# nanoporetech/dorado

Measured on NVIDIA H100. Metric: basecalled samples/s, higher is better.
Workload: dtype f16 (fp32 accumulate; fp32 decode)

## Files before the change

### dorado_b200/csrc/decode.cu

```cuda
#include "decode.h"

#include "b200_crf_math.h"
#include "common.cuh"
#include "engine.h"
#include "nvtx.h"

#include <string>

namespace b200 {

namespace {

constexpr int kBeamW = 32;
constexpr uint32_t kCrcPoly = 0x82f63b78u;
constexpr uint32_t kCrcSeed = 0x12345678u;

template <int SL>
struct Dims {
    static constexpr int S = 1 << (2 * SL);
    static constexpr int C = 4 * S;
};

template <int SL>
struct ScanCfg {
// ... 28 lines not shown
    constexpr int RS = C / 4;
    float* out = bwd + (size_t)chunk_c * (T_pitch + 1) * S;
    const int q = v % P4, top = v / P4;
    const int st_row = 4 * (v & 3), st_col = v >> 2;

    uint2 pf[PF];
#pragma unroll
    for (int k = 0; k < PF; ++k) {
        const int tt = T - 1 - k;
        if (tt >= 0) pf[k] = __ldg(srow + (size_t)tt * RS);
    }
    auto stage = [&](int buf, const uint2& r) {
        const __half2 h0 = *reinterpret_cast<const __half2*>(&r.x), h1 = *reinterpret_cast<const __half2*>(&r.y);
        const float2 f0 = __half22float2(h0), f1 = __half22float2(h1);
        float* d = &st[g][buf][st_row * PITCH + st_col];
        d[0] = clampf(f0.x, clamp_val);
        d[PITCH] = clampf(f0.y, clamp_val);
        d[2 * PITCH] = clampf(f1.x, clamp_val);
        d[3 * PITCH] = clampf(f1.y, clamp_val);
    };
    float own = 0.0f;
    a[g][0][v] = 0.0f;
    if (active) out[(size_t)T * S + v] = 0.0f;
    stage(0, pf[0]);
    if (T - 1 - PF >= 0) pf[0] = __ldg(srow + (size_t)(T - 1 - PF) * RS);
    if constexpr (S <= 32) __syncwarp(); else named_bar_sync(1 + g, S);

    int cur = 0;
    for (int t = T - 1; t >= 0; t -= PF) {
#pragma unroll
        for (int k = 0; k < PF; ++k) {
            const int tt = t - k;
            if (tt >= 0) {
                if (tt - 1 >= 0) {
                    stage(cur ^ 1, pf[(k + 1) % PF]);
                    if (tt - 1 - PF >= 0) pf[(k + 1) % PF] = __ldg(srow + (size_t)(tt - 1 - PF) * RS);
                }
                const float4 nx = *reinterpret_cast<const float4*>(&a[g][cur][4 * q]);
                const float* sc = &st[g][cur][top * PITCH + q];
                own = b200_lse5(B200_ADD(own, blank), B200_ADD(nx.x, sc[0]), B200_ADD(nx.y, sc[4 * PITCH]),
                                B200_ADD(nx.z, sc[8 * PITCH]), B200_ADD(nx.w, sc[12 * PITCH]));
                a[g][cur ^ 1][v] = own;
                if (active) out[(size_t)tt * S + v] = own;
                if constexpr (S <= 32) __syncwarp(); else named_bar_sync(1 + g, S);
                cur ^= 1;
            }
        }
    }
}

__device__ __forceinline__ uint32_t crc_bits(uint32_t crc, uint32_t nb, int nbits) {
    for (int i = 0; i < nbits; ++i) {
        const uint32_t b = (nb ^ crc) & 1u;
        crc >>= 1;
        if (b) crc ^= kCrcPoly;
        nb >>= 1;
    }
    return crc;
}

__device__ __forceinline__ uint32_t crc2(uint32_t crc, uint32_t nb) {
    uint32_t b = (nb ^ crc) & 1u;
    crc = (crc >> 1) ^ (b ? kCrcPoly : 0u);
    b = ((nb >> 1) ^ crc) & 1u;
    crc = (crc >> 1) ^ (b ? kCrcPoly : 0u);
    return crc;
}

__device__ __forceinline__ uint32_t crc2_inv(uint32_t crc, uint32_t nb) {
    uint32_t b = crc >> 31;
    uint32_t t = crc ^ (b ? kCrcPoly : 0u);
    crc = (t << 1) | (b ^ ((nb >> 1) & 1u));
    b = crc >> 31;
    t = crc ^ (b ? kCrcPoly : 0u);
    crc = (t << 1) | (b ^ (nb & 1u));
    return crc;
}

constexpr int kHashSlots = 1024;

struct BeamSmem {
    __align__(16) float cand_score[5 * kBeamW];
    uint32_t cand_hash[5 * kBeamW];
    float new_score[kBeamW];
    uint32_t new_hash[kBeamW];
    uint32_t new_meta[kBeamW];
    __align__(16) uint32_t prev_hash[kBeamW];
    uint8_t slot_lane[kHashSlots];
};

struct BeamLane {
    uint32_t hash;
    uint32_t state;
    float score;
};

__device__ __forceinline__ uint32_t float_key(float f) {
    const uint32_t u = __float_as_uint(f);
    return (u & 0x80000000u) ? ~u : (u | 0x80000000u);
}

template <int SL>
__device__ int beam_init(const float* bw_row, BeamSmem& bs, BeamLane& me, int W, int lane) {
    constexpr int S = Dims<SL>::S;
    constexpr int VPL = S >= 32 ? S / 32 : 1;
    uint32_t keys[VPL];
#pragma unroll
    for (int j = 0; j < VPL; ++j) {
        const int s = lane * VPL + j;
        keys[j] = s < S ? float_key(bw_row[s]) : 0u;
    }
    uint32_t thr = 0u;
    if (W < S) {
        for (int bit = 31; bit >= 0; --bit) {
            const uint32_t cand = thr | (1u << bit);
            int c = 0;
#pragma unroll
            for (int j = 0; j < VPL; ++j) c += (lane * VPL + j < S) && (keys[j] >= cand);
            if (warp_sum_int(c) >= W) thr = cand;
        }
    }
    int c = 0;
#pragma unroll
    for (int j = 0; j < VPL; ++j) c += (lane * VPL + j < S) && (keys[j] >= thr);
    int incl = c;
#pragma unroll
    for (int o = 1; o < 32; o <<= 1) {
        const int v = __shfl_up_sync(0xffffffffu, incl, o);
        if (lane >= o) incl += v;
    }
    int pos = incl - c;
#pragma unroll
    for (int j = 0; j < VPL; ++j) {
        const int s = lane * VPL + j;
        if (s < S && keys[j] >= thr) {
            if (pos < W) bs.new_meta[pos] = (uint32_t)s;
            ++pos;
        }
    }
    __syncwarp();
    const int width = W < S ? W : S;
    if (lane < width) {
        me.state = bs.new_meta[lane] & 0xffffu;
        me.hash = crc_bits(kCrcSeed, me.state, 32);
        me.score = 0.0f;
    }
    __syncwarp();
    return width;
}

template <int SL>
__device__ __forceinline__ float kmer_block_prob(const float* post_row, int state) {
    constexpr int S = Dims<SL>::S;
    float prob = post_row[state];
    const int l = state >> 2;
    const int r = (state << 2) & (S - 1);
    constexpr int msb = S >> 2;
    const int d = l - r;
#pragma unroll
    for (int b = 0; b < 4; ++b) {
        const int L = l + msb * b, R = r + b;
        bool keepL = L != state;
#pragma unroll
        for (int bb = 0; bb < b; ++bb) keepL = keepL && (bb - msb * b != d);
        if (keepL) prob = B200_ADD(prob, post_row[L]);
        bool keepR = R != state;
#pragma unroll
        for (int bb = 0; bb <= b; ++bb) keepR = keepR && (b - msb * bb != d);
        if (keepR) prob = B200_ADD(prob, post_row[R]);
    }
    return prob < 0.0f ? 0.0f : (prob > 1.0f ? 1.0f : prob);
}

template <int SL>
__device__ int beam_step(const __half* sc_row,
                         const float* bw_row,
                         const float* post_row,
                         BeamSmem& bs,
                         BeamLane& me,
                         int width,
                         int W,
                         float log_beam_cut,
                         float blank,
                         bool last_block,
                         uint32_t* meta_row,
                         float* prob_row,
                         int lane,
                         long long* dbg) {
    constexpr int S = Dims<SL>::S;
    constexpr int SB = 2 * SL;
    if (dbg && lane == 0) dbg[0] = clock64();
    constexpr uint32_t mask = S - 1;
    const bool valid = lane < width;
    const uint32_t lt_mask = (1u << lane) - 1u;
    const uint32_t vmask = width >= 32 ? 0xffffffffu : ((1u << width) - 1u);

    uint32_t ns[4], hs[4];
    float s[5];
    float lmax = B200_FLT_LOWEST;
    const uint32_t latest = me.state & 3u;
    const uint32_t target = crc2_inv(me.hash, latest);
    const uint32_t own_slot = me.hash & (kHashSlots - 1);
    if (valid) {
        const uint32_t shifted = me.state << 2;
        const uint32_t dropped = shifted >> SB;
        const uint32_t nb = shifted & mask;
        const float4 bw4 = *reinterpret_cast<const float4*>(bw_row + nb);
        const float bws = bw_row[me.state];
        const float bwv[4] = {bw4.x, bw4.y, bw4.z, bw4.w};
        bs.slot_lane[own_slot] = (uint8_t)lane;
        bs.prev_hash[lane] = me.hash;
#pragma unroll
        for (uint32_t b = 0; b < 4; ++b) {
            ns[b] = nb | b;
            const uint32_t move_idx = ((ns[b] << 2) + dropped) & 0xffffu;
            s[b] = B200_ADD(B200_ADD(me.score, __half2float(sc_row[move_idx])), bwv[b]);
            hs[b] = crc2(me.hash, b);
            lmax = b200_fmaxf(lmax, s[b]);
        }
        s[4] = B200_ADD(B200_ADD(me.score, blank), bws);
        lmax = b200_fmaxf(lmax, s[4]);
        *reinterpret_cast<float4*>(&bs.cand_score[lane * 4]) = make_float4(s[0], s[1], s[2], s[3]);
    }
    float max_score = warp_max(lmax);
    __syncwarp();
    if (dbg && lane == 0) dbg[1] = clock64();

    int jm = -1;
    bool dup = false;
    {
        const uint32_t rb = valid ? bs.slot_lane[own_slot] : (uint32_t)lane;
        const uint32_t c = bs.slot_lane[target & (kHashSlots - 1)] & 31u;
        uint32_t ov = __ballot_sync(0xffffffffu, valid && rb != (uint32_t)lane);
        if (valid && ((vmask >> c) & 1u) && bs.prev_hash[c] == target) jm = (int)c;
        while (ov) {
            const int j = __ffs(ov) - 1;
            ov &= ov - 1;
            const uint32_t hj = __shfl_sync(0xffffffffu, me.hash, j);
            if (valid && lane != j && me.hash == hj) dup = true;
            if (valid && target == hj) jm = j;
        }
    }
    if (!__any_sync(0xffffffffu, dup)) {
        float folded = B200_FLT_LOWEST;
        if (jm >= 0) {
            const int pi = jm * 4 + (int)latest;
            const float st = s[4], sp = bs.cand_score[pi];
            folded = b200_log_sum_exp(st, sp);
            if (st > sp) {
                s[4] = folded;
                bs.cand_score[pi] = B200_FLT_LOWEST;
            } else {
                bs.cand_score[pi] = folded;
                s[4] = B200_FLT_LOWEST;
            }
        }
        max_score = b200_fmaxf(max_score, warp_max(folded));
        __syncwarp();
        if (valid) {
            const float4 r = *reinterpret_cast<const float4*>(&bs.cand_score[lane * 4]);
            s[0] = r.x; s[1] = r.y; s[2] = r.z; s[3] = r.w;
        }
    } else {
        if (valid) {
#pragma unroll
            for (int b = 0; b < 4; ++b) bs.cand_hash[lane * 4 + b] = hs[b];
            bs.cand_score[4 * width + lane] = s[4];
            bs.cand_hash[4 * width + lane] = me.hash;
        }
        bs.new_meta[lane] = valid ? latest : 0u;
        __syncwarp();
        float m2 = max_score;
        if (lane == 0) {
            for (int i = 0; i < width; ++i) {
                const int si = 4 * width + i;
                const int lt = (int)bs.new_meta[i];
                for (int j = 0; j < width; ++j) {
                    const int pi = j * 4 + lt;
                    if (bs.cand_hash[si] == bs.cand_hash[pi]) {
                        const float st = bs.cand_score[si], sp = bs.cand_score[pi];
                        const float folded = b200_log_sum_exp(st, sp);
                        if (st > sp) {
                            bs.cand_score[si] = folded;
                            bs.cand_score[pi] = B200_FLT_LOWEST;
                        } else {
                            bs.cand_score[pi] = folded;
                            bs.cand_score[si] = B200_FLT_LOWEST;
                        }
                        m2 = b200_fmaxf(m2, folded);
                    }
                }
            }
        }
        max_score = __shfl_sync(0xffffffffu, m2, 0);
        __syncwarp();
        if (valid) {
#pragma unroll
            for (int b = 0; b < 4; ++b) s[b] = bs.cand_score[lane * 4 + b];
            s[4] = bs.cand_score[4 * width + lane];
        }
        __syncwarp();
    }

    if (dbg && lane == 0) dbg[2] = clock64();
    auto count_part = [&](float c) {
        int n = 0;
        if (valid) {
#pragma unroll
            for (int k = 0; k < 5; ++k) n += (s[k] >= c);
        }
        return n;
    };
    float cutoff = B200_SUB(max_score, log_beam_cut);
    int cnt = warp_sum_int(count_part(cutoff));
    if (cnt > W) {
        const int min_w = (W * 8) / 10;
        float lo = cutoff, hi = max_score;
        int guesses = 1;
        while ((cnt > W || cnt < min_w) && guesses < 10) {
            if (cnt > W) {
                lo = cutoff;
                cutoff = B200_MUL(B200_ADD(cutoff, hi), 0.5f);
            } else {
                hi = cutoff;
                cutoff = B200_MUL(B200_ADD(cutoff, lo), 0.5f);
            }
            cnt = warp_sum_int(count_part(cutoff));
            ++guesses;
        }
        if (guesses == 10) {
            cutoff = hi;
            cnt = warp_sum_int(count_part(cutoff));
        }
        if (cnt > W) cnt = W;
    }

    if (dbg && lane == 0) dbg[3] = clock64();
    bool f[5];
#pragma unroll
    for (int k = 0; k < 5; ++k) f[k] = valid && (s[k] >= cutoff);
    const uint32_t b0 = __ballot_sync(0xffffffffu, f[0]), b1 = __ballot_sync(0xffffffffu, f[1]);
    const uint32_t b2 = __ballot_sync(0xffffffffu, f[2]), b3 = __ballot_sync(0xffffffffu, f[3]);
    const uint32_t b4 = __ballot_sync(0xffffffffu, f[4]);
    int pos = __popc(b0 & lt_mask) + __popc(b1 & lt_mask) + __popc(b2 & lt_mask) + __popc(b3 & lt_mask);
    const int steps_total = __popc(b0) + __popc(b1) + __popc(b2) + __popc(b3);
#pragma unroll
    for (int b = 0; b < 4; ++b) {
        if (f[b]) {
            if (pos < W) {
                bs.new_score[pos] = s[b];
                bs.new_hash[pos] = hs[b];
                bs.new_meta[pos] = ns[b] | ((uint32_t)lane << 16);
            }
            ++pos;
        }
    }
    if (f[4]) {
        const int sp = steps_total + __popc(b4 & lt_mask);
        if (sp < W) {
            bs.new_score[sp] = s[4];
            bs.new_hash[sp] = me.hash;
            bs.new_meta[sp] = me.state | ((uint32_t)lane << 16) | (1u << 24);
        }
    }
    __syncwarp();

    const bool nvalid = lane < cnt;
    uint32_t meta = 0;
    if (nvalid) {
        me.score = bs.new_score[lane];
        me.hash = bs.new_hash[lane];
        meta = bs.new_meta[lane];
        me.state = meta & 0xffffu;
    }

    if (dbg && lane == 0) dbg[4] = clock64();
    if (last_block) {
        const float best = warp_max(nvalid ? me.score : B200_FLT_LOWEST);
        const uint32_t eq = __ballot_sync(0xffffffffu, nvalid && me.score == best && best > B200_FLT_LOWEST);
        const int bi = eq ? (__ffs(eq) - 1) : 0;
        const int src = lane == 0 ? bi : (lane == bi ? 0 : lane);
        const float sc2 = __shfl_sync(0xffffffffu, me.score, src);
        const uint32_t h2 = __shfl_sync(0xffffffffu, me.hash, src);
        const uint32_t m2 = __shfl_sync(0xffffffffu, meta, src);
        me.score = sc2;
        me.hash = h2;
        meta = m2;
        me.state = meta & 0xffffu;
    }
    if (nvalid) {
        me.score = B200_SUB(me.score, bw_row[me.state]);
        meta_row[lane] = meta;
        prob_row[lane] = kmer_block_prob<SL>(post_row, (int)me.state);
    }
    __syncwarp();
    if (dbg && lane == 0) {
        dbg[5] = clock64();
        dbg[6] = cnt;
    }
    return cnt;
}

__device__ __forceinline__ void named_bar_arrive(int id, int nthreads) {
    asm volatile("bar.arrive %0, %1;" ::"r"(id), "r"(nthreads) : "memory");
}

template <int SL>
struct FwdCfg {
    using Scan = ScanCfg<SL>;
    static constexpr int GT = Scan::NT + 32;
    static constexpr int CH = GT <= 128 ? 2 : 1;
    static constexpr int THREADS = GT * CH;
};

template <int SL>
__global__ void __launch_bounds__(FwdCfg<SL>::THREADS) crf_fwd_beam_kernel(const __half* __restrict__ scores,
                                                                          const float* __restrict__ bwd,
                                                                          uint2* __restrict__ beam,
                                                                          int N,
                                                                          int T_pitch,
                                                                          float clamp_val,
                                                                          float blank,
                                                                          int W,
                                                                          float log_beam_cut,
                                                                          const int32_t* __restrict__ lens,
                                                                          int stride,
                                                                          long long* dbg) {
    using Cfg = ScanCfg<SL>;
    using F = FwdCfg<SL>;
    constexpr int S = Cfg::S, C = Cfg::C, P4 = Cfg::P4, SPT = Cfg::SPT, NT = Cfg::NT;
    constexpr int GT = F::GT, CH = F::CH;
    constexpr int NW = NT / 32;
    constexpr int PF = 4;

    const int g = threadIdx.x / GT;
    const int tid = threadIdx.x % GT;
    const int lane = threadIdx.x & 31;
    const int chunk = blockIdx.x * CH + g;
    const int BAR_SCAN = 1 + 5 * g, BAR_FULL = 2 + 5 * g, BAR_EMPTY = 4 + 5 * g;

    __shared__ __align__(16) float fa[CH][2][S];
    __shared__ __align__(16) __half sc_row[CH][2][C];
    __shared__ __align__(16) float bw_row[CH][2][S];
    __shared__ __align__(16) float post_row[CH][2][S];
    __shared__ float red[CH][2][NW];
    __shared__ BeamSmem bsm[CH];

    if (chunk >= N) return;
    const int T = lens ? min(T_pitch, __ldg(lens + chunk) / stride) : T_pitch;
    uint32_t* meta_out = reinterpret_cast<uint32_t*>(beam) + (size_t)chunk * T_pitch * kBeamW;
    float* prob_out = reinterpret_cast<float*>(beam) + ((size_t)N + chunk) * T_pitch * kBeamW;

    if (tid < NT) {
        const int v = tid;
        const int wv = v >> 5;
// ... 33 lines not shown
                    if (t >= 2) named_bar_sync(BAR_EMPTY + slot, GT);
                    if (d) d[9] = clock64();
                    float vsum[SPT];
                    float lmax = B200_FLT_LOWEST;
#pragma unroll
                    for (int e = 0; e < SPT; ++e) {
                        const uint2 r = pf[k][e];
                        const float bw = pb[k][e];
                        if (t + PF < T) {
                            pf[k][e] = __ldg(reinterpret_cast<const uint2*>(srow + (size_t)(t + PF) * C) + e);
                            pb[k][e] = __ldg(brow + (size_t)(t + PF + 1) * S + e);
                        }
                        const float2 f0 = __half22float2(*reinterpret_cast<const __half2*>(&r.x));
                        const float2 f1 = __half22float2(*reinterpret_cast<const __half2*>(&r.y));
                        const float s0 = clampf(f0.x, clamp_val), s1 = clampf(f0.y, clamp_val);
                        const float s2 = clampf(f1.x, clamp_val), s3 = clampf(f1.y, clamp_val);
                        const int st = SPT * v + e;
                        {
                            const __half2 c0 = __floats2half2_rn(s0, s1), c1 = __floats2half2_rn(s2, s3);
                            uint2 pk;
                            pk.x = *reinterpret_cast<const uint32_t*>(&c0);
                            pk.y = *reinterpret_cast<const uint32_t*>(&c1);
                            *reinterpret_cast<uint2*>(&sc_row[g][slot][4 * st]) = pk;
                        }
                        bw_row[g][slot][st] = bw;
                        const int p = st >> 2;
                        f[e] = b200_lse5(B200_ADD(f[e], blank), B200_ADD(fa[g][cur][p], s0), B200_ADD(fa[g][cur][p + P4], s1),
                                         B200_ADD(fa[g][cur][p + 2 * P4], s2), B200_ADD(fa[g][cur][p + 3 * P4], s3));
                        fa[g][cur ^ 1][st] = f[e];
                        vsum[e] = B200_ADD(f[e], bw);
                        lmax = b200_fmaxf(lmax, vsum[e]);
                    }
                    float mx = warp_max(lmax);
                    if constexpr (NW > 1) {
                        if (lane == 0) red[g][0][wv] = mx;
                        named_bar_sync(BAR_SCAN, NT);
                        mx = red[g][0][0];
#pragma unroll
                        for (int w = 1; w < NW; ++w) mx = b200_fmaxf(mx, red[g][0][w]);
                    }
                    float ex[SPT];
                    float part = 0.0f;
#pragma unroll
                    for (int e = 0; e < SPT; ++e) {
                        ex[e] = b200_expf_nonpos(B200_SUB(vsum[e], mx));
                        part = e == 0 ? ex[0] : B200_ADD(part, ex[e]);
                    }
#pragma unroll
                    for (int o = 16; o >= 1; o >>= 1) part = B200_ADD(part, __shfl_xor_sync(0xffffffffu, part, o));
                    float z = part;
                    if constexpr (NW > 1) {
                        if (lane == 0) red[g][1][wv] = part;
                        named_bar_sync(BAR_SCAN, NT);
                        z = red[g][1][0];
#pragma unroll
                        for (int w = 1; w < NW; ++w) z = B200_ADD(z, red[g][1][w]);
                    }
#pragma unroll
                    for (int e = 0; e < SPT; ++e) post_row[g][slot][SPT * v + e] = B200_DIV(ex[e], z);
                    named_bar_arrive(BAR_FULL + slot, GT);
                    if (d) d[10] = clock64();
                    cur ^= 1;
                }
            }
        }
    } else {
        named_bar_sync(BAR_SCAN, GT);
        BeamLane me{0u, 0u, 0.0f};
        int width = beam_init<SL>(bw_row[g][1], bsm[g], me, W, lane);
        named_bar_sync(BAR_SCAN, GT);
        for (int t = 0; t < T; ++t) {
            const int slot = t & 1;
            long long* d = (dbg && chunk == 0 && t >= 100 && t < 108) ? dbg + (t - 100) * 16 : nullptr;
            if (d && lane == 0) d[7] = clock64();
            named_bar_sync(BAR_FULL + slot, GT);
            width = beam_step<SL>(sc_row[g][slot], bw_row[g][slot], post_row[g][slot], bsm[g], me, width, W, log_beam_cut, blank,
                                  t == T - 1, meta_out + (size_t)t * kBeamW, prob_out + (size_t)t * kBeamW, lane, d);
            if (t + 2 < T) named_bar_arrive(BAR_EMPTY + slot, GT);
        }
    }
}

constexpr int kWarpDecodeMaxChunks = 16;
constexpr int kWarpStPitch = 16 + 2;

struct WarpDecodeSmem {
    __align__(16) float fa[2][64];
    float st[16 * kWarpStPitch];
    __align__(16) __half sc_row[256];
    __align__(16) float bw_row[64];
    __align__(16) float post_row[64];
    BeamSmem bs;
};

__device__ __forceinline__ float4 clamped_scores(const uint2& r, float clamp_val) {
    const float2 f0 = __half22float2(*reinterpret_cast<const __half2*>(&r.x));
    const float2 f1 = __half22float2(*reinterpret_cast<const __half2*>(&r.y));
    return make_float4(clampf(f0.x, clamp_val), clampf(f0.y, clamp_val), clampf(f1.x, clamp_val), clampf(f1.y, clamp_val));
}

__global__ void __launch_bounds__(kWarpDecodeMaxChunks * 32, 1) crf_decode_warp_kernel(const __half* __restrict__ scores,
                                                                                      float* __restrict__ bwd,
                                                                                      uint2* __restrict__ beam,
                                                                                      int N,
                                                                                      int T_pitch,
                                                                                      float clamp_val,
                                                                                      float blank,
                                                                                      int W,
                                                                                      float log_beam_cut,
                                                                                      const int32_t* __restrict__ lens,
                                                                                      int stride) {
    constexpr int S = Dims<3>::S, C = Dims<3>::C, P4 = S / 4, PITCH = kWarpStPitch;
    constexpr int RS = C / 4;
    constexpr int PF = 4;
    extern __shared__ __align__(16) unsigned char warp_decode_smem[];
    const int w = threadIdx.x >> 5, lane = threadIdx.x & 31;
    const int chunk = blockIdx.x * (blockDim.x >> 5) + w;
    if (chunk >= N) return;
    WarpDecodeSmem& sm = reinterpret_cast<WarpDecodeSmem*>(warp_decode_smem)[w];
    const int T = lens ? min(T_pitch, __ldg(lens + chunk) / stride) : T_pitch;
    const uint2* srow = reinterpret_cast<const uint2*>(scores + (size_t)chunk * T_pitch * C);
    float* brow = bwd + (size_t)chunk * (T_pitch + 1) * S;
    const int s0 = lane, s1 = lane + 32;

    {
        const int q = lane & 15, top = lane >> 4;
        auto stage = [&](const uint2& r, int v) {
            const float4 f = clamped_scores(r, clamp_val);
            float* d = &sm.st[4 * (v & 3) * PITCH + (v >> 2)];
            d[0] = f.x;
            d[PITCH] = f.y;
            d[2 * PITCH] = f.z;
            d[3 * PITCH] = f.w;
        };
        uint2 pf[PF][2];
#pragma unroll
        for (int k = 0; k < PF; ++k) {
            const int tt = T - 1 - k;
            if (tt >= 0) {
                pf[k][0] = __ldg(srow + (size_t)tt * RS + s0);
                pf[k][1] = __ldg(srow + (size_t)tt * RS + s1);
            }
        }
        float own0 = 0.0f, own1 = 0.0f;
        sm.fa[0][s0] = 0.0f;
        sm.fa[0][s1] = 0.0f;
        brow[(size_t)T * S + s0] = 0.0f;
        brow[(size_t)T * S + s1] = 0.0f;
        int cur = 0;
        for (int t = T - 1; t >= 0; t -= PF) {
#pragma unroll
            for (int k = 0; k < PF; ++k) {
                const int tt = t - k;
                if (tt >= 0) {
                    stage(pf[k][0], s0);
                    stage(pf[k][1], s1);
                    if (tt - PF >= 0) {
                        pf[k][0] = __ldg(srow + (size_t)(tt - PF) * RS + s0);
                        pf[k][1] = __ldg(srow + (size_t)(tt - PF) * RS + s1);
                    }
                    __syncwarp();
                    const float4 nx = *reinterpret_cast<const float4*>(&sm.fa[cur][4 * q]);
                    const float* sa = &sm.st[top * PITCH + q];
                    const float* sb = &sm.st[(top + 2) * PITCH + q];
                    own0 = b200_lse5(B200_ADD(own0, blank), B200_ADD(nx.x, sa[0]), B200_ADD(nx.y, sa[4 * PITCH]),
                                     B200_ADD(nx.z, sa[8 * PITCH]), B200_ADD(nx.w, sa[12 * PITCH]));
                    own1 = b200_lse5(B200_ADD(own1, blank), B200_ADD(nx.x, sb[0]), B200_ADD(nx.y, sb[4 * PITCH]),
                                     B200_ADD(nx.z, sb[8 * PITCH]), B200_ADD(nx.w, sb[12 * PITCH]));
                    sm.fa[cur ^ 1][s0] = own0;
                    sm.fa[cur ^ 1][s1] = own1;
                    brow[(size_t)tt * S + s0] = own0;
                    brow[(size_t)tt * S + s1] = own1;
                    __syncwarp();
                    cur ^= 1;
                }
            }
        }
    }
    __syncwarp();

    uint32_t* meta_out = reinterpret_cast<uint32_t*>(beam) + (size_t)chunk * T_pitch * kBeamW;
    float* prob_out = reinterpret_cast<float*>(beam) + ((size_t)N + chunk) * T_pitch * kBeamW;
    sm.fa[0][s0] = 0.0f;
    sm.fa[0][s1] = 0.0f;
    sm.bw_row[s0] = brow[s0];
    sm.bw_row[s1] = brow[s1];
    __syncwarp();
    BeamLane me{0u, 0u, 0.0f};
    int width = beam_init<3>(sm.bw_row, sm.bs, me, W, lane);
    uint2 r0n{}, r1n{};
    float b0n = 0.0f, b1n = 0.0f;
    if (T > 0) {
        r0n = __ldg(srow + s0);
        r1n = __ldg(srow + s1);
        b0n = brow[S + s0];
        b1n = brow[S + s1];
    }
    float f0 = 0.0f, f1 = 0.0f;
    int cur = 0;
    const int p0 = s0 >> 2, p1 = s1 >> 2;
    for (int t = 0; t < T; ++t) {
        const uint2 r0 = r0n, r1 = r1n;
        const float bw0 = b0n, bw1 = b1n;
        if (t + 1 < T) {
            r0n = __ldg(srow + (size_t)(t + 1) * RS + s0);
            r1n = __ldg(srow + (size_t)(t + 1) * RS + s1);
            b0n = brow[(size_t)(t + 2) * S + s0];
            b1n = brow[(size_t)(t + 2) * S + s1];
        }
        const float4 c0 = clamped_scores(r0, clamp_val), c1 = clamped_scores(r1, clamp_val);
        {
            const __half2 h00 = __floats2half2_rn(c0.x, c0.y), h01 = __floats2half2_rn(c0.z, c0.w);
            const __half2 h10 = __floats2half2_rn(c1.x, c1.y), h11 = __floats2half2_rn(c1.z, c1.w);
            *reinterpret_cast<uint2*>(&sm.sc_row[4 * s0]) =
                    make_uint2(*reinterpret_cast<const uint32_t*>(&h00), *reinterpret_cast<const uint32_t*>(&h01));
            *reinterpret_cast<uint2*>(&sm.sc_row[4 * s1]) =
                    make_uint2(*reinterpret_cast<const uint32_t*>(&h10), *reinterpret_cast<const uint32_t*>(&h11));
        }
        sm.bw_row[s0] = bw0;
        sm.bw_row[s1] = bw1;
        const float* fc = sm.fa[cur];
        f0 = b200_lse5(B200_ADD(f0, blank), B200_ADD(fc[p0], c0.x), B200_ADD(fc[p0 + P4], c0.y), B200_ADD(fc[p0 + 2 * P4], c0.z),
                       B200_ADD(fc[p0 + 3 * P4], c0.w));
        f1 = b200_lse5(B200_ADD(f1, blank), B200_ADD(fc[p1], c1.x), B200_ADD(fc[p1 + P4], c1.y), B200_ADD(fc[p1 + 2 * P4], c1.z),
                       B200_ADD(fc[p1 + 3 * P4], c1.w));
        sm.fa[cur ^ 1][s0] = f0;
        sm.fa[cur ^ 1][s1] = f1;
        const float v0 = B200_ADD(f0, bw0), v1 = B200_ADD(f1, bw1);
        const float mx = warp_max(b200_fmaxf(v0, v1));
        const float e0 = b200_expf_nonpos(B200_SUB(v0, mx)), e1 = b200_expf_nonpos(B200_SUB(v1, mx));
        float z0 = e0, z1 = e1;
#pragma unroll
        for (int o = 16; o >= 1; o >>= 1) {
            z0 = B200_ADD(z0, __shfl_xor_sync(0xffffffffu, z0, o));
            z1 = B200_ADD(z1, __shfl_xor_sync(0xffffffffu, z1, o));
        }
        const float z = B200_ADD(z0, z1);
        sm.post_row[s0] = B200_DIV(e0, z);
        sm.post_row[s1] = B200_DIV(e1, z);
        __syncwarp();
        width = beam_step<3>(sm.sc_row, sm.bw_row, sm.post_row, sm.bs, me, width, W, log_beam_cut, blank, t == T - 1,
                             meta_out + (size_t)t * kBeamW, prob_out + (size_t)t * kBeamW, lane, nullptr);
        cur ^= 1;
    }
}

int warp_decode_chunks_per_cta(int N, int runners) {
    const int R = runners > 1 ? runners : 1;
    const int per = (int)(((long long)N * R + kNumSMs - 1) / kNumSMs);
    return per < 1 ? 1 : (per > kWarpDecodeMaxChunks ? kWarpDecodeMaxChunks : per);
}

constexpr int kTbTile = 32;
constexpr int kTbWarps = 2;

__host__ __device__ constexpr size_t traceback_warp_bytes(int T) {
    return ((size_t)kTbTile * kBeamW * 4 + (size_t)((T + 3) & ~3) * (4 + 4 + 2) + 16 + 15) & ~(size_t)15;
}

__global__ void __launch_bounds__(kTbWarps * 32) crf_traceback_kernel(const uint32_t* __restrict__ beam_meta,
                                                                      const float* __restrict__ beam_prob,
                                                                      int N,
                                                                      int T_pitch,
                                                                      const int32_t* __restrict__ lens,
                                                                      int stride,
                                                                      const b200_qtable* __restrict__ qtable,
                                                                      uint8_t* __restrict__ moves_out,
                                                                      char* __restrict__ seq_out,
                                                                      char* __restrict__ qstr_out,
                                                                      int32_t* __restrict__ n_bases_out) {
    extern __shared__ __align__(16) unsigned char tb_smem[];
    __shared__ b200_qtable qt;
    for (int i = threadIdx.x; i < (int)(sizeof(b200_qtable) / 4); i += blockDim.x) {
        reinterpret_cast<uint32_t*>(&qt)[i] = reinterpret_cast<const uint32_t*>(qtable)[i];
    }
    __syncthreads();
    const int w = threadIdx.x >> 5, lane = threadIdx.x & 31;
    const int chunk = blockIdx.x * kTbWarps + w;
    if (chunk >= N) return;
    const int T = lens ? min(T_pitch, __ldg(lens + chunk) / stride) : T_pitch;
    const int Tp = (T_pitch + 3) & ~3;
    unsigned char* base = tb_smem + (size_t)w * traceback_warp_bytes(T_pitch);
    uint32_t* tile = reinterpret_cast<uint32_t*>(base);
    uint32_t* path = tile + kTbTile * kBeamW;
    float* pprob = reinterpret_cast<float*>(path + Tp);
    uint16_t* bstart = reinterpret_cast<uint16_t*>(pprob + Tp);

    const uint32_t* mrow = beam_meta + (size_t)chunk * T_pitch * kBeamW + lane;
    uint32_t nxt[kTbTile];
    auto load_tile = [&](int t_hi) {
        const int t_lo = t_hi - kTbTile;
#pragma unroll
        for (int r = 0; r < kTbTile; ++r) {
            const int t = t_lo + r;
            nxt[r] = t >= 0 ? __ldg(mrow + (size_t)t * kBeamW) : 0u;
        }
    };
    if (T > 0) load_tile(T);
    uint32_t ei = 0;
    for (int t_hi = T; t_hi > 0; t_hi -= kTbTile) {
#pragma unroll
        for (int r = 0; r < kTbTile; ++r) tile[r * kBeamW + lane] = nxt[r];
        __syncwarp();
        if (t_hi - kTbTile > 0) load_tile(t_hi - kTbTile);
        if (lane == 0) {
            const int t_lo = t_hi - kTbTile;
            const int r_lo = t_lo < 0 ? -t_lo : 0;
            for (int r = kTbTile - 1; r >= r_lo; --r) {
                const uint32_t e = tile[r * kBeamW + ei];
                path[t_lo + r] = (e & 0xffffu) | ((((e >> 24) & 1u) ^ 1u) << 16) | (ei << 24);
                ei = (e >> 16) & 0xffu;
            }
        }
        __syncwarp();
    }
    if (lane == 0 && T > 0) path[0] |= 1u << 16;
    __syncwarp();
    {
        const float* prow = beam_prob + (size_t)chunk * T_pitch * kBeamW;
        for (int t = lane; t < T; t += 32) {
            pprob[t] = b200_pow0p4f(__ldg(prow + (size_t)t * kBeamW + (path[t] >> 24)));
        }
    }
    __syncwarp();

    int nb = 0;
    for (int t0 = 0; t0 < T; t0 += 32) {
        const int t = t0 + lane;
        const bool m = t < T && ((path[t] >> 16) & 1u);
        const uint32_t bal = __ballot_sync(0xffffffffu, m);
        if (m) bstart[nb + __popc(bal & ((1u << lane) - 1u))] = (uint16_t)t;
        nb += __popc(bal);
    }
    if (lane == 0) bstart[nb] = (uint16_t)T;
    __syncwarp();

    uint8_t* mo = moves_out + (size_t)chunk * T_pitch;
    char* so = seq_out + (size_t)chunk * T_pitch;
    char* qo = qstr_out + (size_t)chunk * T_pitch;
    for (int t = lane; t < T_pitch; t += 32) mo[t] = t < T ? (uint8_t)((path[t] >> 16) & 1u) : 0;
    for (int p = lane; p < T_pitch; p += 32) {
        char sc = 0, qc = 0;
        if (p < nb) {
            const int b0 = bstart[p], b1 = bstart[p + 1];
            float bp = 0.0f, tp = 0.0f;
            int base = 0;
            for (int blk = b0; blk < b1; ++blk) {
                base = path[blk] & 3;
                const float prob = pprob[blk];
                const float wrong = B200_DIV(B200_SUB(1.0f, prob), 3.0f);
                bp = B200_ADD(bp, prob);
#pragma unroll
                for (int k = 0; k < 4; ++k) tp = B200_ADD(tp, k == base ? prob : wrong);
            }
            sc = "ACGT"[path[b0] & 3];
            qc = b200_qtable_lookup(&qt, bp, tp);
        }
        so[p] = sc;
        qo[p] = qc;
    }
    if (lane == 0) n_bases_out[chunk] = nb;
}

size_t traceback_smem_bytes(int T) { return kTbWarps * traceback_warp_bytes(T); }

void launch_traceback(const DecodeArgs& a, cudaStream_t stream, ProfileSink* prof) {
    const size_t smem = traceback_smem_bytes(a.T);
    if (smem > 48 * 1024) ensure_dynamic_smem(crf_traceback_kernel, 200 * 1024);
    const int grid = (a.N + kTbWarps - 1) / kTbWarps;
    NvtxRange r("decode");
    const uint32_t* meta = reinterpret_cast<const uint32_t*>(a.beam);
    const float* prob = reinterpret_cast<const float*>(a.beam) + (size_t)a.N * a.T * kBeamW;
    crf_traceback_kernel<<<grid, kTbWarps * 32, smem, stream>>>(meta, prob, a.N, a.T, a.lens, a.stride, a.qtable, a.moves,
                                                                a.sequence, a.qstring, a.n_bases);
    if (prof) prof->mark("crf_traceback", stream);
}

void launch_decode_warp(const DecodeArgs& a, cudaStream_t stream, ProfileSink* prof) {
    {
        const int cpc = warp_decode_chunks_per_cta(a.N, a.runners);
        const int grid = (a.N + cpc - 1) / cpc;
        const size_t smem = (size_t)cpc * sizeof(WarpDecodeSmem);
        ensure_dynamic_smem(crf_decode_warp_kernel, (int)(kWarpDecodeMaxChunks * sizeof(WarpDecodeSmem)));
        NvtxRange r("beam_search");
        crf_decode_warp_kernel<<<grid, cpc * 32, smem, stream>>>(a.scores, a.bwd, a.beam, a.N, a.T, a.clamp_val, a.blank,
                                                                 a.beam_width, a.log_beam_cut, a.lens, a.stride);
        if (prof) prof->mark("crf_fwd_beam", stream);
    }
    launch_traceback(a, stream, prof);
    B200_CUDA(cudaGetLastError());
}

template <int SL>
void launch_decode(const DecodeArgs& a, cudaStream_t stream, ProfileSink* prof) {
    {
        constexpr int S = Dims<SL>::S;
        constexpr int CH = S >= 256 ? 1 : 256 / S;
        const int grid = (a.N + CH - 1) / CH;
        NvtxRange r("back_guides");
        crf_bwd_scan_kernel<SL><<<grid, S * CH, 0, stream>>>(a.scores, a.bwd, a.N, a.T, a.clamp_val, a.blank, a.lens, a.stride);
        if (prof) prof->mark("crf_bwd_scan", stream);
    }
    {
        using F = FwdCfg<SL>;
        const int grid = (a.N + F::CH - 1) / F::CH;
        NvtxRange r("beam_search");
        crf_fwd_beam_kernel<SL><<<grid, F::THREADS, 0, stream>>>(a.scores, a.bwd, a.beam, a.N, a.T, a.clamp_val, a.blank,
                                                                   a.beam_width, a.log_beam_cut, a.lens, a.stride, a.dbg);
        if (prof) prof->mark("crf_fwd_beam", stream);
    }
    launch_traceback(a, stream, prof);
    B200_CUDA(cudaGetLastError());
}

}

size_t decode_max_blocks() {
    int T = 65535;
    while (traceback_smem_bytes(T) > 200 * 1024) T -= 64;
    return (size_t)T;
}

void carve_decode_scratch(Bump& b, int N, int T, int state_len, float** bwd, uint2** beam) {
    const size_t S = (size_t)1 << (2 * state_len);
    *bwd = b.take<float>((size_t)N * (T + 1) * S * sizeof(float));
    *beam = b.take<uint2>((size_t)N * T * kBeamW * sizeof(uint2));
}

int decode_launches(int state_len) { return state_len == 3 ? 2 : 3; }

void decode_scores(const DecodeArgs& a, cudaStream_t stream, ProfileSink* prof) {
    if (a.beam_width < 1 || a.beam_width > kBeamW) {
        throw std::invalid_argument("b200 decode: beam_width must be in [1, 32]");
    }
    if (a.T < 1 || a.T > 65535 || a.N < 1) {
        throw std::invalid_argument("b200 decode: need 1 <= T <= 65535 and N >= 1");
    }
    if (!a.qtable) throw std::invalid_argument("b200 decode: quality table missing");
    if (a.lens && a.stride < 1) throw std::invalid_argument("b200 decode: chunk lengths need the model stride");
    if (traceback_smem_bytes(a.T) > 200 * 1024) {
        throw std::invalid_argument("b200 decode: " + std::to_string(a.T) + " blocks per chunk exceed what the traceback kernel "
                                    "holds in shared memory (about 10 700); use a smaller chunk size");
    }
    switch (a.state_len) {
        case 3: launch_decode_warp(a, stream, prof); break;
        case 4: launch_decode<4>(a, stream, prof); break;
        case 5: launch_decode<5>(a, stream, prof); break;
        default: throw std::invalid_argument("b200 decode: state_len must be 3, 4 or 5");
    }
}

}
```

### include/b200_crf_math.h

```cpp
#ifndef B200_CRF_MATH_H
#define B200_CRF_MATH_H

#include <stdint.h>

#if defined(__CUDA_ARCH__)
#define B200_MATH_FN static __device__ __forceinline__
#define B200_FMA(a, b, c) __fmaf_rn((a), (b), (c))
#define B200_MUL(a, b) __fmul_rn((a), (b))
#define B200_ADD(a, b) __fadd_rn((a), (b))
#define B200_SUB(a, b) __fsub_rn((a), (b))
#define B200_DIV(a, b) __fdiv_rn((a), (b))
#define B200_F2U(x) __float_as_uint(x)
#define B200_U2F(x) __uint_as_float(x)
#else
#include <math.h>
#include <string.h>
#define B200_MATH_FN static inline
#define B200_FMA(a, b, c) fmaf((a), (b), (c))
#define B200_MUL(a, b) ((a) * (b))
#define B200_ADD(a, b) ((a) + (b))
#define B200_SUB(a, b) ((a) - (b))
#define B200_DIV(a, b) ((a) / (b))
static inline uint32_t b200_f2u_(float x) {
    uint32_t u;
    memcpy(&u, &x, 4);
    return u;
}
static inline float b200_u2f_(uint32_t u) {
    float x;
    memcpy(&x, &u, 4);
    return x;
}
#define B200_F2U(x) b200_f2u_(x)
#define B200_U2F(x) b200_u2f_(x)
#endif

#define B200_FLT_LOWEST (-3.402823466e+38f)

B200_MATH_FN float b200_fmaxf(float a, float b) { return a > b ? a : b; }

B200_MATH_FN float b200_expf(float x) {
    const float xc = x < -86.0f ? -86.0f : (x > 88.0f ? 88.0f : x);
    const float t = B200_MUL(xc, 1.44269504088896341f);
    const float big = 12582912.0f;
    const float tb = B200_ADD(t, big);
    const float n = B200_SUB(tb, big);
    float r = B200_FMA(n, -0.693359375f, xc);
    r = B200_FMA(n, 2.12194440e-4f, r);
    float p = 1.9875691500e-4f;
    p = B200_FMA(p, r, 1.3981999507e-3f);
    p = B200_FMA(p, r, 8.3334519073e-3f);
    p = B200_FMA(p, r, 4.1665795894e-2f);
    p = B200_FMA(p, r, 1.6666665459e-1f);
    p = B200_FMA(p, r, 5.0000001201e-1f);
    const float r2 = B200_MUL(r, r);
    p = B200_FMA(p, r2, r);
    p = B200_ADD(p, 1.0f);
    const float scale = B200_U2F((B200_F2U(tb) << 23) + 0x3f800000u);
    const float y = B200_MUL(p, scale);
    return x < -86.0f ? 0.0f : y;
}

B200_MATH_FN float b200_expf_nonpos(float x) {
    const float xc = x < -86.0f ? -86.0f : x;
    const float t = B200_MUL(xc, 1.44269504088896341f);
    const float big = 12582912.0f;
    const float tb = B200_ADD(t, big);
    const float n = B200_SUB(tb, big);
    float r = B200_FMA(n, -0.693359375f, xc);
    r = B200_FMA(n, 2.12194440e-4f, r);
    float p = 1.9875691500e-4f;
    p = B200_FMA(p, r, 1.3981999507e-3f);
    p = B200_FMA(p, r, 8.3334519073e-3f);
    p = B200_FMA(p, r, 4.1665795894e-2f);
    p = B200_FMA(p, r, 1.6666665459e-1f);
    p = B200_FMA(p, r, 5.0000001201e-1f);
    const float r2 = B200_MUL(r, r);
    p = B200_FMA(p, r2, r);
    p = B200_ADD(p, 1.0f);
    const float scale = B200_U2F((B200_F2U(tb) << 23) + 0x3f800000u);
    const float y = B200_MUL(p, scale);
    return x < -86.0f ? 0.0f : y;
}

B200_MATH_FN float b200_logf(float x) {
    const uint32_t ix = B200_F2U(x);
    int32_t e = (int32_t)((ix >> 23) & 0xffu) - 126;
    float m = B200_U2F((ix & 0x007fffffu) | 0x3f000000u);
    if (m < 0.707106781186547524f) {
        e -= 1;
        m = B200_SUB(B200_ADD(m, m), 1.0f);
    } else {
        m = B200_SUB(m, 1.0f);
    }
    const float z = B200_MUL(m, m);
    float y = 7.0376836292e-2f;
    y = B200_FMA(y, m, -1.1514610310e-1f);
    y = B200_FMA(y, m, 1.1676998740e-1f);
    y = B200_FMA(y, m, -1.2420140846e-1f);
    y = B200_FMA(y, m, 1.4249322787e-1f);
    y = B200_FMA(y, m, -1.6668057665e-1f);
    y = B200_FMA(y, m, 2.0000714765e-1f);
    y = B200_FMA(y, m, -2.4999993993e-1f);
    y = B200_FMA(y, m, 3.3333331174e-1f);
    y = B200_MUL(B200_MUL(y, m), z);
    const float fe = (float)e;
    y = B200_FMA(fe, -2.12194440e-4f, y);
    y = B200_FMA(z, -0.5f, y);
    float r = B200_ADD(m, y);
    r = B200_FMA(fe, 0.693359375f, r);
    return r;
}

B200_MATH_FN float b200_log1pf(float x) {
    const float u = B200_ADD(1.0f, x);
    const float c = B200_SUB(x, B200_SUB(u, 1.0f));
    return B200_ADD(b200_logf(u), B200_DIV(c, u));
}

B200_MATH_FN float b200_log_sum_exp(float x, float y) {
    const float d = B200_SUB(x, y);
    const float ad = d < 0.0f ? -d : d;
    const float mx = b200_fmaxf(x, y);
    if (ad < 17.0f) {
        return B200_ADD(mx, b200_log1pf(b200_expf(-ad)));
    }
    return mx;
}

B200_MATH_FN float b200_lse5(float v_stay, float v0, float v1, float v2, float v3) {
    float m = b200_fmaxf(v_stay, v0);
    m = b200_fmaxf(m, v1);
    m = b200_fmaxf(m, v2);
    m = b200_fmaxf(m, v3);
    float s = b200_expf_nonpos(B200_SUB(v_stay, m));
    s = B200_ADD(s, b200_expf_nonpos(B200_SUB(v0, m)));
    s = B200_ADD(s, b200_expf_nonpos(B200_SUB(v1, m)));
    s = B200_ADD(s, b200_expf_nonpos(B200_SUB(v2, m)));
    s = B200_ADD(s, b200_expf_nonpos(B200_SUB(v3, m)));
    return B200_ADD(m, b200_logf(s));
}

#if defined(__CUDA_ARCH__)
#define B200_DFMA(a, b, c) __fma_rn((a), (b), (c))
#define B200_DMUL(a, b) __dmul_rn((a), (b))
#define B200_DADD(a, b) __dadd_rn((a), (b))
#define B200_DSUB(a, b) __dsub_rn((a), (b))
#define B200_DDIV(a, b) __ddiv_rn((a), (b))
#define B200_D2U(x) ((uint64_t)__double_as_longlong(x))
#define B200_U2D(x) __longlong_as_double((long long)(x))
#define B200_D2F(x) __double2float_rn(x)
#else
#define B200_DFMA(a, b, c) fma((a), (b), (c))
#define B200_DMUL(a, b) ((a) * (b))
#define B200_DADD(a, b) ((a) + (b))
#define B200_DSUB(a, b) ((a) - (b))
#define B200_DDIV(a, b) ((a) / (b))
static inline uint64_t b200_d2u_(double x) {
    uint64_t u;
    memcpy(&u, &x, 8);
    return u;
}
static inline double b200_u2d_(uint64_t u) {
    double x;
    memcpy(&x, &u, 8);
    return x;
}
#define B200_D2U(x) b200_d2u_(x)
#define B200_U2D(x) b200_u2d_(x)
#define B200_D2F(x) ((float)(x))
#endif

B200_MATH_FN float b200_pow0p4f(float p) {
    if (p <= 0.0f) {
        return 0.0f;
    }
    if (p >= 1.0f) {
        return 1.0f;
    }
    const double x = (double)p;
    const uint64_t ix = B200_D2U(x);
    int64_t e = (int64_t)((ix >> 52) & 0x7ffu) - 1023;
    double m = B200_U2D((ix & 0x000fffffffffffffull) | 0x3ff0000000000000ull);
    if (m > 1.4142135623730951) {
        m = B200_DMUL(m, 0.5);
        e += 1;
    }
    const double s = B200_DDIV(B200_DSUB(m, 1.0), B200_DADD(m, 1.0));
    const double s2 = B200_DMUL(s, s);
    double q = 1.0 / 23.0;
    q = B200_DFMA(q, s2, 1.0 / 21.0);
    q = B200_DFMA(q, s2, 1.0 / 19.0);
    q = B200_DFMA(q, s2, 1.0 / 17.0);
    q = B200_DFMA(q, s2, 1.0 / 15.0);
    q = B200_DFMA(q, s2, 1.0 / 13.0);
    q = B200_DFMA(q, s2, 1.0 / 11.0);
    q = B200_DFMA(q, s2, 1.0 / 9.0);
    q = B200_DFMA(q, s2, 1.0 / 7.0);
    q = B200_DFMA(q, s2, 1.0 / 5.0);
    q = B200_DFMA(q, s2, 1.0 / 3.0);
    double lm = B200_DFMA(B200_DMUL(s, s2), q, s);
    lm = B200_DADD(lm, lm);
    const double fe = (double)e;
    double lx = B200_DFMA(fe, 1.90821492927058770002e-10, lm);
    lx = B200_DFMA(fe, 6.93147180369123816490e-01, lx);
    const double y = B200_DMUL(lx, 0.4000000059604644775390625);
    const double t = B200_DMUL(y, 1.44269504088896338700e+00);
    const double big = 6755399441055744.0;
    const double n = B200_DSUB(B200_DADD(t, big), big);
    double r = B200_DFMA(n, -6.93147180369123816490e-01, y);
    r = B200_DFMA(n, -1.90821492927058770002e-10, r);
    double ex = 1.0 / 6227020800.0;
    ex = B200_DFMA(ex, r, 1.0 / 479001600.0);
    ex = B200_DFMA(ex, r, 1.0 / 39916800.0);
    ex = B200_DFMA(ex, r, 1.0 / 3628800.0);
    ex = B200_DFMA(ex, r, 1.0 / 362880.0);
    ex = B200_DFMA(ex, r, 1.0 / 40320.0);
// ... 90 lines not shown
```

Before: 1.099 billion.

## Streamline CRF warp decode: register-resident backward scores, packed beam smem, half clamp

The backward pass now loads scores with 128-bit loads and uses byte_perm to pick each lane's pairs in registers. This drops the shared-memory transpose staging buffer and a per-step syncwarp. Beam candidates are packed into one uint4 array so each lane does a single vector store and load. The kernel is templated to clamp in half precision when the clamp value is exactly representable in fp16. Several micro-optimisations are bundled in: CRC hashes via linearity (crc2(h,0) xor crc2(0,b)), branch-free expf underflow via a -88 clamp, and hardware fmaxf in lse5. These risk small numerical differences, for example NaN handling in fmaxf and the tiny underflow values of expf.

Result: faster. 1.126 billion (median of 6 runs) (+2.5%).

```diff
diff --git a/dorado_b200/csrc/decode.cu b/dorado_b200/csrc/decode.cu
--- a/dorado_b200/csrc/decode.cu
+++ b/dorado_b200/csrc/decode.cu
@@ -134,9 +134,7 @@
 struct BeamSmem {
     __align__(16) float cand_score[5 * kBeamW];
     uint32_t cand_hash[5 * kBeamW];
-    float new_score[kBeamW];
-    uint32_t new_hash[kBeamW];
-    uint32_t new_meta[kBeamW];
+    uint4 kept[kBeamW];
     __align__(16) uint32_t prev_hash[kBeamW];
     uint8_t slot_lane[kHashSlots];
 };
@@ -186,14 +184,14 @@
     for (int j = 0; j < VPL; ++j) {
         const int s = lane * VPL + j;
         if (s < S && keys[j] >= thr) {
-            if (pos < W) bs.new_meta[pos] = (uint32_t)s;
+            if (pos < W) bs.kept[pos].z = (uint32_t)s;
             ++pos;
         }
     }
     __syncwarp();
     const int width = W < S ? W : S;
     if (lane < width) {
-        me.state = bs.new_meta[lane] & 0xffffu;
+        me.state = bs.kept[lane].z & 0xffffu;
         me.hash = crc_bits(kCrcSeed, me.state, 32);
         me.score = 0.0f;
     }
@@ -251,7 +249,8 @@
     float s[5];
     float lmax = B200_FLT_LOWEST;
     const uint32_t latest = me.state & 3u;
-    const uint32_t target = crc2_inv(me.hash, latest);
+    const uint32_t target = crc2_inv(me.hash, 0u) ^ latest;
+    const uint32_t hash0 = crc2(me.hash, 0u);
     const uint32_t own_slot = me.hash & (kHashSlots - 1);
     if (valid) {
         const uint32_t shifted = me.state << 2;
@@ -267,7 +266,7 @@
             ns[b] = nb | b;
             const uint32_t move_idx = ((ns[b] << 2) + dropped) & 0xffffu;
             s[b] = B200_ADD(B200_ADD(me.score, __half2float(sc_row[move_idx])), bwv[b]);
-            hs[b] = crc2(me.hash, b);
+            hs[b] = hash0 ^ crc2(0u, b);
             lmax = b200_fmaxf(lmax, s[b]);
         }
         s[4] = B200_ADD(B200_ADD(me.score, blank), bws);
@@ -320,13 +319,13 @@
             bs.cand_score[4 * width + lane] = s[4];
             bs.cand_hash[4 * width + lane] = me.hash;
         }
-        bs.new_meta[lane] = valid ? latest : 0u;
+        bs.kept[lane].z = valid ? latest : 0u;
         __syncwarp();
         float m2 = max_score;
         if (lane == 0) {
             for (int i = 0; i < width; ++i) {
                 const int si = 4 * width + i;
-                const int lt = (int)bs.new_meta[i];
+                const int lt = (int)bs.kept[i].z;
                 for (int j = 0; j < width; ++j) {
                     const int pi = j * 4 + lt;
                     if (bs.cand_hash[si] == bs.cand_hash[pi]) {
@@ -399,30 +398,23 @@
 #pragma unroll
     for (int b = 0; b < 4; ++b) {
         if (f[b]) {
-            if (pos < W) {
-                bs.new_score[pos] = s[b];
-                bs.new_hash[pos] = hs[b];
-                bs.new_meta[pos] = ns[b] | ((uint32_t)lane << 16);
-            }
+            if (pos < W) bs.kept[pos] = make_uint4(__float_as_uint(s[b]), hs[b], ns[b] | ((uint32_t)lane << 16), 0u);
             ++pos;
         }
     }
     if (f[4]) {
         const int sp = steps_total + __popc(b4 & lt_mask);
-        if (sp < W) {
-            bs.new_score[sp] = s[4];
-            bs.new_hash[sp] = me.hash;
-            bs.new_meta[sp] = me.state | ((uint32_t)lane << 16) | (1u << 24);
-        }
+        if (sp < W) bs.kept[sp] = make_uint4(__float_as_uint(s[4]), me.hash, me.state | ((uint32_t)lane << 16) | (1u << 24), 0u);
     }
     __syncwarp();
 
     const bool nvalid = lane < cnt;
     uint32_t meta = 0;
     if (nvalid) {
-        me.score = bs.new_score[lane];
-        me.hash = bs.new_hash[lane];
-        meta = bs.new_meta[lane];
+        const uint4 k = bs.kept[lane];
+        me.score = __uint_as_float(k.x);
+        me.hash = k.y;
+        meta = k.z;
         me.state = meta & 0xffffu;
     }
 
@@ -622,23 +614,50 @@
 }
 
 constexpr int kWarpDecodeMaxChunks = 16;
-constexpr int kWarpStPitch = 16 + 2;
 
 struct WarpDecodeSmem {
     __align__(16) float fa[2][64];
-    float st[16 * kWarpStPitch];
     __align__(16) __half sc_row[256];
     __align__(16) float bw_row[64];
     __align__(16) float post_row[64];
     BeamSmem bs;
 };
 
-__device__ __forceinline__ float4 clamped_scores(const uint2& r, float clamp_val) {
-    const float2 f0 = __half22float2(*reinterpret_cast<const __half2*>(&r.x));
-    const float2 f1 = __half22float2(*reinterpret_cast<const __half2*>(&r.y));
-    return make_float4(clampf(f0.x, clamp_val), clampf(f0.y, clamp_val), clampf(f1.x, clamp_val), clampf(f1.y, clamp_val));
-}
-
+__device__ __forceinline__ __half2 half_clamp_bound(float clamp_val) {
+    return __float2half2_rn(clamp_val > 0.0f ? clamp_val : __int_as_float(0x7f800000));
+}
+
+template <bool kHalfClamp>
+__device__ __forceinline__ float2 clamp_pair(uint32_t w, float clamp_val, __half2 bound) {
+    __half2 h = *reinterpret_cast<const __half2*>(&w);
+    if constexpr (kHalfClamp) {
+        return __half22float2(__hmin2(__hmax2(h, __hneg2(bound)), bound));
+    } else {
+        const float2 f = __half22float2(h);
+        return make_float2(clampf(f.x, clamp_val), clampf(f.y, clamp_val));
+    }
+}
+
+template <bool kHalfClamp>
+__device__ __forceinline__ float4 clamp_scores(uint2& r, float clamp_val, __half2 bound) {
+    __half2 h0 = *reinterpret_cast<const __half2*>(&r.x), h1 = *reinterpret_cast<const __half2*>(&r.y);
+    if constexpr (kHalfClamp) {
+        h0 = __hmin2(__hmax2(h0, __hneg2(bound)), bound);
+        h1 = __hmin2(__hmax2(h1, __hneg2(bound)), bound);
+        r = make_uint2(*reinterpret_cast<const uint32_t*>(&h0), *reinterpret_cast<const uint32_t*>(&h1));
+        const float2 f0 = __half22float2(h0), f1 = __half22float2(h1);
+        return make_float4(f0.x, f0.y, f1.x, f1.y);
+    } else {
+        const float2 f0 = __half22float2(h0), f1 = __half22float2(h1);
+        const float4 c = make_float4(clampf(f0.x, clamp_val), clampf(f0.y, clamp_val), clampf(f1.x, clamp_val),
+                                     clampf(f1.y, clamp_val));
+        const __half2 c0 = __floats2half2_rn(c.x, c.y), c1 = __floats2half2_rn(c.z, c.w);
+        r = make_uint2(*reinterpret_cast<const uint32_t*>(&c0), *reinterpret_cast<const uint32_t*>(&c1));
+        return c;
+    }
+}
+
+template <bool kHalfClamp>
 __global__ void __launch_bounds__(kWarpDecodeMaxChunks * 32, 1) crf_decode_warp_kernel(const __half* __restrict__ scores,
                                                                                       float* __restrict__ bwd,
                                                                                       uint2* __restrict__ beam,
@@ -650,7 +669,7 @@
                                                                                       float log_beam_cut,
                                                                                       const int32_t* __restrict__ lens,
                                                                                       int stride) {
-    constexpr int S = Dims<3>::S, C = Dims<3>::C, P4 = S / 4, PITCH = kWarpStPitch;
+    constexpr int S = Dims<3>::S, C = Dims<3>::C, P4 = S / 4;
     constexpr int RS = C / 4;
     constexpr int PF = 4;
     extern __shared__ __align__(16) unsigned char warp_decode_smem[];
@@ -662,24 +681,21 @@
     const uint2* srow = reinterpret_cast<const uint2*>(scores + (size_t)chunk * T_pitch * C);
     float* brow = bwd + (size_t)chunk * (T_pitch + 1) * S;
     const int s0 = lane, s1 = lane + 32;
+    const __half2 bound = half_clamp_bound(clamp_val);
 
     {
         const int q = lane & 15, top = lane >> 4;
-        auto stage = [&](const uint2& r, int v) {
-            const float4 f = clamped_scores(r, clamp_val);
-            float* d = &sm.st[4 * (v & 3) * PITCH + (v >> 2)];
-            d[0] = f.x;
-            d[PITCH] = f.y;
-            d[2 * PITCH] = f.z;
-            d[3 * PITCH] = f.w;
-        };
-        uint2 pf[PF][2];
+        const uint4* qrow = reinterpret_cast<const uint4*>(srow) + 2 * q;
+        constexpr int RQ = C / 8;
+        const uint32_t sel = top ? 0x7632u : 0x5410u;
+        auto pair = [&](uint32_t lo, uint32_t hi) { return clamp_pair<kHalfClamp>(__byte_perm(lo, hi, sel), clamp_val, bound); };
+        uint4 pf[PF][2];
 #pragma unroll
         for (int k = 0; k < PF; ++k) {
             const int tt = T - 1 - k;
             if (tt >= 0) {
-                pf[k][0] = __ldg(srow + (size_t)tt * RS + s0);
-                pf[k][1] = __ldg(srow + (size_t)tt * RS + s1);
+                pf[k][0] = __ldg(qrow + (size_t)tt * RQ);
+                pf[k][1] = __ldg(qrow + (size_t)tt * RQ + 1);
             }
         }
         float own0 = 0.0f, own1 = 0.0f;
@@ -687,26 +703,24 @@
         sm.fa[0][s1] = 0.0f;
         brow[(size_t)T * S + s0] = 0.0f;
         brow[(size_t)T * S + s1] = 0.0f;
+        __syncwarp();
         int cur = 0;
         for (int t = T - 1; t >= 0; t -= PF) {
 #pragma unroll
             for (int k = 0; k < PF; ++k) {
                 const int tt = t - k;
                 if (tt >= 0) {
-                    stage(pf[k][0], s0);
-                    stage(pf[k][1], s1);
+                    const uint4 a = pf[k][0], b = pf[k][1];
                     if (tt - PF >= 0) {
-                        pf[k][0] = __ldg(srow + (size_t)(tt - PF) * RS + s0);
-                        pf[k][1] = __ldg(srow + (size_t)(tt - PF) * RS + s1);
+                        pf[k][0] = __ldg(qrow + (size_t)(tt - PF) * RQ);
+                        pf[k][1] = __ldg(qrow + (size_t)(tt - PF) * RQ + 1);
                     }
-                    __syncwarp();
+                    const float2 m0 = pair(a.x, a.y), m1 = pair(a.z, a.w), m2 = pair(b.x, b.y), m3 = pair(b.z, b.w);
                     const float4 nx = *reinterpret_cast<const float4*>(&sm.fa[cur][4 * q]);
-                    const float* sa = &sm.st[top * PITCH + q];
-                    const float* sb = &sm.st[(top + 2) * PITCH + q];
-                    own0 = b200_lse5(B200_ADD(own0, blank), B200_ADD(nx.x, sa[0]), B200_ADD(nx.y, sa[4 * PITCH]),
-                                     B200_ADD(nx.z, sa[8 * PITCH]), B200_ADD(nx.w, sa[12 * PITCH]));
-                    own1 = b200_lse5(B200_ADD(own1, blank), B200_ADD(nx.x, sb[0]), B200_ADD(nx.y, sb[4 * PITCH]),
-                                     B200_ADD(nx.z, sb[8 * PITCH]), B200_ADD(nx.w, sb[12 * PITCH]));
+                    own0 = b200_lse5(B200_ADD(own0, blank), B200_ADD(nx.x, m0.x), B200_ADD(nx.y, m1.x), B200_ADD(nx.z, m2.x),
+                                     B200_ADD(nx.w, m3.x));
+                    own1 = b200_lse5(B200_ADD(own1, blank), B200_ADD(nx.x, m0.y), B200_ADD(nx.y, m1.y), B200_ADD(nx.z, m2.y),
+                                     B200_ADD(nx.w, m3.y));
                     sm.fa[cur ^ 1][s0] = own0;
                     sm.fa[cur ^ 1][s1] = own1;
                     brow[(size_t)tt * S + s0] = own0;
@@ -740,7 +754,7 @@
     int cur = 0;
     const int p0 = s0 >> 2, p1 = s1 >> 2;
     for (int t = 0; t < T; ++t) {
-        const uint2 r0 = r0n, r1 = r1n;
+        uint2 r0 = r0n, r1 = r1n;
         const float bw0 = b0n, bw1 = b1n;
         if (t + 1 < T) {
             r0n = __ldg(srow + (size_t)(t + 1) * RS + s0);
@@ -748,15 +762,9 @@
             b0n = brow[(size_t)(t + 2) * S + s0];
             b1n = brow[(size_t)(t + 2) * S + s1];
         }
-        const float4 c0 = clamped_scores(r0, clamp_val), c1 = clamped_scores(r1, clamp_val);
-        {
-            const __half2 h00 = __floats2half2_rn(c0.x, c0.y), h01 = __floats2half2_rn(c0.z, c0.w);
-            const __half2 h10 = __floats2half2_rn(c1.x, c1.y), h11 = __floats2half2_rn(c1.z, c1.w);
-            *reinterpret_cast<uint2*>(&sm.sc_row[4 * s0]) =
-                    make_uint2(*reinterpret_cast<const uint32_t*>(&h00), *reinterpret_cast<const uint32_t*>(&h01));
-            *reinterpret_cast<uint2*>(&sm.sc_row[4 * s1]) =
-                    make_uint2(*reinterpret_cast<const uint32_t*>(&h10), *reinterpret_cast<const uint32_t*>(&h11));
-        }
+        const float4 c0 = clamp_scores<kHalfClamp>(r0, clamp_val, bound), c1 = clamp_scores<kHalfClamp>(r1, clamp_val, bound);
+        *reinterpret_cast<uint2*>(&sm.sc_row[4 * s0]) = r0;
+        *reinterpret_cast<uint2*>(&sm.sc_row[4 * s1]) = r1;
         sm.bw_row[s0] = bw0;
         sm.bw_row[s1] = bw1;
         const float* fc = sm.fa[cur];
@@ -921,10 +929,12 @@
         const int cpc = warp_decode_chunks_per_cta(a.N, a.runners);
         const int grid = (a.N + cpc - 1) / cpc;
         const size_t smem = (size_t)cpc * sizeof(WarpDecodeSmem);
-        ensure_dynamic_smem(crf_decode_warp_kernel, (int)(kWarpDecodeMaxChunks * sizeof(WarpDecodeSmem)));
+        const bool half_clamp = !(a.clamp_val > 0.0f) || __half2float(__float2half_rn(a.clamp_val)) == a.clamp_val;
+        auto kernel = half_clamp ? crf_decode_warp_kernel<true> : crf_decode_warp_kernel<false>;
+        ensure_dynamic_smem(kernel, (int)(kWarpDecodeMaxChunks * sizeof(WarpDecodeSmem)));
         NvtxRange r("beam_search");
-        crf_decode_warp_kernel<<<grid, cpc * 32, smem, stream>>>(a.scores, a.bwd, a.beam, a.N, a.T, a.clamp_val, a.blank,
-                                                                 a.beam_width, a.log_beam_cut, a.lens, a.stride);
+        kernel<<<grid, cpc * 32, smem, stream>>>(a.scores, a.bwd, a.beam, a.N, a.T, a.clamp_val, a.blank, a.beam_width,
+                                                 a.log_beam_cut, a.lens, a.stride);
         if (prof) prof->mark("crf_fwd_beam", stream);
     }
     launch_traceback(a, stream, prof);
diff --git a/include/b200_crf_math.h b/include/b200_crf_math.h
--- a/include/b200_crf_math.h
+++ b/include/b200_crf_math.h
@@ -40,7 +40,7 @@
 B200_MATH_FN float b200_fmaxf(float a, float b) { return a > b ? a : b; }
 
 B200_MATH_FN float b200_expf(float x) {
-    const float xc = x < -86.0f ? -86.0f : (x > 88.0f ? 88.0f : x);
+    const float xc = x < -86.0f ? -88.0f : (x > 88.0f ? 88.0f : x);
     const float t = B200_MUL(xc, 1.44269504088896341f);
     const float big = 12582912.0f;
     const float tb = B200_ADD(t, big);
@@ -57,12 +57,11 @@
     p = B200_FMA(p, r2, r);
     p = B200_ADD(p, 1.0f);
     const float scale = B200_U2F((B200_F2U(tb) << 23) + 0x3f800000u);
-    const float y = B200_MUL(p, scale);
-    return x < -86.0f ? 0.0f : y;
+    return B200_MUL(p, scale);
 }
 
 B200_MATH_FN float b200_expf_nonpos(float x) {
-    const float xc = x < -86.0f ? -86.0f : x;
+    const float xc = x < -86.0f ? -88.0f : x;
     const float t = B200_MUL(xc, 1.44269504088896341f);
     const float big = 12582912.0f;
     const float tb = B200_ADD(t, big);
@@ -79,8 +78,7 @@
     p = B200_FMA(p, r2, r);
     p = B200_ADD(p, 1.0f);
     const float scale = B200_U2F((B200_F2U(tb) << 23) + 0x3f800000u);
-    const float y = B200_MUL(p, scale);
-    return x < -86.0f ? 0.0f : y;
+    return B200_MUL(p, scale);
 }
 
 B200_MATH_FN float b200_logf(float x) {
@@ -120,7 +118,7 @@
 
 B200_MATH_FN float b200_log_sum_exp(float x, float y) {
     const float d = B200_SUB(x, y);
-    const float ad = d < 0.0f ? -d : d;
+    const float ad = fabsf(d);
     const float mx = b200_fmaxf(x, y);
     if (ad < 17.0f) {
         return B200_ADD(mx, b200_log1pf(b200_expf(-ad)));
@@ -128,11 +126,17 @@
     return mx;
 }
 
+#if defined(__CUDA_ARCH__)
+#define B200_LSE_MAX(a, b) fmaxf((a), (b))
+#else
+#define B200_LSE_MAX(a, b) b200_fmaxf((a), (b))
+#endif
+
 B200_MATH_FN float b200_lse5(float v_stay, float v0, float v1, float v2, float v3) {
-    float m = b200_fmaxf(v_stay, v0);
-    m = b200_fmaxf(m, v1);
-    m = b200_fmaxf(m, v2);
-    m = b200_fmaxf(m, v3);
+    float m = B200_LSE_MAX(v_stay, v0);
+    m = B200_LSE_MAX(m, v1);
+    m = B200_LSE_MAX(m, v2);
+    m = B200_LSE_MAX(m, v3);
     float s = b200_expf_nonpos(B200_SUB(v_stay, m));
     s = B200_ADD(s, b200_expf_nonpos(B200_SUB(v0, m)));
     s = B200_ADD(s, b200_expf_nonpos(B200_SUB(v1, m)));
```
